# pfnet-research/superpixel-align

Measured on AMD Instinct MI355X. Metric: images/sec superpixel-align labelling (1024x2048), higher is better.
Workload: dtype f32 as 2 x f16 planes, f32 accumulate

## Files before the change

### include/spalign.h

```cpp
#ifndef SPALIGN_H
#define SPALIGN_H

#include <stddef.h>
#include <stdint.h>

#ifdef __cplusplus
extern "C" {
#endif

#define SPA_OK 0
#define SPA_ERR_ARG (-1)
#define SPA_ERR_HIP (-2)
#define SPA_ERR_NOGPU (-3)
#define SPA_ERR_LAYOUT (-4)
#define SPA_ERR_CAPACITY (-5)

#define SPA_ST_SLIC_EMPTY_SEGMENT 0x01u
#define SPA_ST_SLIC_UNCOVERED 0x02u
#define SPA_ST_CONN_OVERSIZE 0x04u
#define SPA_ST_POOL_SLOT_OVERFLOW 0x08u
#define SPA_ST_KMEANS_BARRIER 0x10u
#define SPA_ST_LABEL_RANGE 0x20u
#define SPA_ST_RNG_UNDERRUN 0x40u
#define SPA_ST_NP_SHUFFLE 0x80u
// ... 6 lines not shown
const char *spa_last_error(void);
int spa_ctx_create(int device, spa_ctx **out);
void spa_ctx_destroy(spa_ctx *ctx);
int spa_status(spa_ctx *ctx, uint32_t *status_host, void *stream);
int spa_status_peek_async(spa_ctx *ctx, uint32_t *status_pinned, void *stream);
int spa_status_take_async(spa_ctx *ctx, uint32_t *status_pinned, void *stream);

int spa_prof_enable(spa_ctx *ctx, int on);
int spa_prof_slots(void);
const char *spa_prof_name(int slot);
int spa_prof_read(spa_ctx *ctx, int slot, double *total_ms_host, int *launches_host);
int spa_debug_peek(spa_ctx *ctx, int which, size_t offset, size_t bytes, void *host);
int spa_ws_generation(spa_ctx *ctx);
int spa_debug_set(spa_ctx *ctx, int32_t key, int32_t value);
int spa_wino4_tile_decode(int32_t B, int32_t H, int32_t W, int32_t dilation, int32_t interleaved, int64_t t, int32_t *out);
int spa_debug_lds_probe(spa_ctx *ctx, float *out, int32_t n_wg, int32_t steps, int32_t mode, void *stream);

int spa_drn_normalise(spa_ctx *ctx, const float *x, int32_t B, int32_t H, int32_t W, void *out,
                      int32_t out_dtype, const double *mean3_host, const double *std3_host, void *stream);
int spa_bias_act(spa_ctx *ctx, void *y, int32_t dtype, int64_t rows, int32_t C, const void *bias,
                 const void *residual, int32_t relu, void *stream);
int spa_bias_act_amax(spa_ctx *ctx, float *y, int64_t rows, int32_t C, const float *bias,
                      const float *residual, int32_t relu, void *amax, void *stream);

int spa_drn_stem_d(spa_ctx *ctx, const float *x, int32_t B, int32_t H, int32_t W,
                   const float *w0, const float *b0, const float *w1, const float *b1,
                   const double *mean3_host, const double *std3_host, void *y, int32_t out_dtype,
                   float *xn_scratch, void *stream);

int spa_conv3x3_bf16(spa_ctx *ctx, const void *x, int32_t B, int32_t H, int32_t W, int32_t Cin,
// ... 281 lines not shown
```

### superpixel-align_amd/_lib.py

```python
import ctypes
import os
import subprocess

_HERE = os.path.dirname(os.path.abspath(__file__))
LIB_PATH = os.environ.get('SPA_LIB_PATH') or os.path.join(_HERE, 'libspalign.so')
_LIB = None

SPA_OK = 0
STATUS_BITS = {
    0x01: 'SLIC: a seed lost all of its pixels (NaN centre, dead for the rest of the sweeps, as in scikit-image)',
    0x02: 'SLIC: a pixel fell outside every 2S search window',
    0x04: 'connectivity: a component reached max_size (cut in BFS order by the exact replay path)',
    0x08: 'mean pooling: more than 16 superpixels touch one feature pixel',
    0x10: 'k-means: grid barrier timed out',
    0x20: 'a superpixel label outside [0, n_labels) was met',
    0x40: 'anchor selection: the device random stream ran dry',
    0x80: 'k-means initial assignment on the device: more than 65 536 points at or below the median weight',
}

INFO_BITS = 0x01 | 0x04

c_i32 = ctypes.c_int32
c_i64 = ctypes.c_int64
c_f32 = ctypes.c_float
# ... 44 lines not shown
    'spa_bias_act_amax': (ctypes.c_int, [c_p, c_p, c_i64, c_i32, c_p, c_p, c_i32, c_p, c_p]),
    'spa_drn_stem_d_amax': (ctypes.c_int, [c_p, c_p, c_i32, c_i32, c_i32, c_p, c_p, c_p, c_p, c_p, c_p, c_p, c_p, c_p, c_p]),
    'spa_drn_stem_c_amax': (ctypes.c_int, [c_p, c_p, c_i32, c_i32, c_i32, c_p, c_p, c_p, c_p, c_p, c_p, c_p, c_p, c_p, c_p, c_p]),
    'spa_drn_stem_c_bf16': (ctypes.c_int, [c_p, c_p, c_i32, c_i32, c_i32, c_p, c_p, c_p, c_p, c_p, c_p, c_p, c_p, c_p, c_p]),
    'spa_conv_small_f16s': (ctypes.c_int, [c_p, c_p, c_i32, c_i32, c_i32, c_i32, c_p, c_f32, c_i32, c_i32, c_i32, c_p, c_p, c_i32, c_p, c_p, c_p, c_p, c_p]),
    'spa_drn_layer2_f16s': (ctypes.c_int, [c_p, c_p, c_i32, c_i32, c_i32, c_p, c_f32, c_p, c_p, c_p, c_p, c_p]),
    'spa_drn_layer2_f32': (ctypes.c_int, [c_p, c_p, c_i32, c_i32, c_i32, c_p, c_p, c_p, c_p]),
    'spa_conv3x3_s2_f32': (ctypes.c_int, [c_p, c_p, c_i32, c_i32, c_i32, c_i32, c_p, c_i32, c_i32, c_p, c_i32, c_p, c_p, c_p]),
    'spa_amax_f32': (ctypes.c_int, [c_p, c_p, c_i64, c_p, c_p]),
    'spa_conv3x3_wino4_f16s': (ctypes.c_int, [c_p, c_p, c_i32, c_i32, c_i32, c_i32, c_p, c_p, c_i32, c_p, c_p, c_i32, c_i32, c_p, c_p, c_p, c_p, c_p, c_p]),
    'spa_resize_bicubic_u8': (ctypes.c_int, [c_p, c_p, c_i32, c_i32, c_i32, c_i32, c_i32, c_i32, c_p, c_p]),
    'spa_resize_cvcubic_u8': (ctypes.c_int, [c_p, c_p, c_i32, c_i32, c_i32, c_i32, c_i32, c_i32, c_p, c_p]),
    'spa_debug_peek': (ctypes.c_int, [c_p, ctypes.c_int, ctypes.c_size_t, ctypes.c_size_t, c_p]),
    'spa_debug_set': (ctypes.c_int, [c_p, ctypes.c_int32, ctypes.c_int32]),
    'spa_wino4_tile_decode': (ctypes.c_int, [c_i32, c_i32, c_i32, c_i32, c_i32, c_i64, ctypes.POINTER(ctypes.c_int32)]),
    'spa_ws_generation': (ctypes.c_int, [c_p]),
    'spa_debug_lds_probe': (ctypes.c_int, [c_p, c_p, c_i32, c_i32, c_i32, c_p]),
    'spa_slic_make_plan':(ctypes.c_int, [c_i32, c_i32, c_i32, ctypes.POINTER(SlicPlan)]),
    'spa_rgb2lab': (ctypes.c_int, [c_p, c_p, c_i32, c_i32, c_i32, c_f32, c_p, c_p]),
    'spa_slic_core': (ctypes.c_int, [c_p, c_p, c_i32, c_i32, c_i32, c_i32, c_i32, c_p, c_p, c_p]),
    'spa_enforce_connectivity': (ctypes.c_int, [c_p, c_p, c_i32, c_i32, c_i32, c_i32, c_i32, c_p,
                                                c_p, c_p]),
    'spa_slic': (ctypes.c_int, [c_p, c_p, c_i32, c_i32, c_i32, c_i32, c_f32, c_i32, c_p, c_p, c_p]),
    'spa_felzenszwalb': (ctypes.c_int, [c_p, c_p, c_i32, c_i32, c_i32, c_f64, c_f64, c_i32, c_p, c_p, c_p]),
    'spa_rgb2lab_u8_f64': (ctypes.c_int, [c_p, c_p, c_i32, c_i32, c_i32, c_f64, c_p, c_p]),
    'spa_slic_core_f64': (ctypes.c_int, [c_p, c_p, c_i32, c_i32, c_i32, c_i32, c_i32, c_p, c_p, c_p]),
    'spa_slic_u8': (ctypes.c_int, [c_p, c_p, c_i32, c_i32, c_i32, c_i32, c_f64, c_i32, c_p, c_p, c_p]),
    'spa_felzenszwalb_u8': (ctypes.c_int, [c_p, c_p, c_i32, c_i32, c_i32, c_f64, c_f64, c_i32, c_p, c_p, c_p]),
    'spa_overlap_refine': (ctypes.c_int, [c_p, c_p, c_p, c_i32, c_i64, c_i32, c_f64, c_p, c_p]),
    'spa_segment_offsets':(ctypes.c_int, [c_p, c_p, c_i32, c_p, c_p]),
# ... 111 lines not shown
```

### superpixel-align_amd/csrc/spa_common.h

```cpp
#pragma once
#include <hip/hip_runtime.h>
#include <stdint.h>
#include <stdio.h>
#include <string.h>

#include "../../include/spalign.h"

#define SPA_WAVE 64

void spa_set_error(const char *fmt, ...);

#define SPA_HIP(call)                                                                  \
    do {                                                                               \
        hipError_t e_ = (call);                                                        \
        if (e_ != hipSuccess) {                                                        \
            spa_set_error("%s failed: %s (%s:%d)", #call, hipGetErrorString(e_),      \
                          __FILE__, __LINE__);                                         \
            return SPA_ERR_HIP;                                                        \
        }                                                                              \
    } while (0)

#define SPA_ARG(cond)                                                                  \
    do {                                                                               \
        if (!(cond)) {                                                                 \
// ... 80 lines not shown
    hipStream_t aux[2];
    hipEvent_t ev_fork, ev_join[2];
    int aux_ready;
    int km_attr_done[2];
    int conn_attr_done;
    int conn_claim_ready;
    size_t conn_claim_bytes;
    int upd_wg_per_cu, upd_wg_per_cu8;
    int slic_force_general;
    int zero_line_ready, conv_attr_done, conv32_attr_done, fz_attr_done, gemm16_attr_done, gemm16s_attr_done, gemm16p_attr_done, nprng_attr_done;
    int rng_seeded;
    int ws_generation;
    int dbg_slic_ldsx;
    int convp_on;
    int wino_operands;
    int convs2_on;
    int convs2_attr_done;
    int rs_key[4], rs_ks[2];
};

#ifdef __HIPCC__
__device__ __forceinline__ unsigned spa_split16_pair(float x0, float x1, float sc, unsigned &l)
{
    unsigned h, lo;
    asm("v_fma_mixlo_f16 %0, %2, %4, 0 op_sel_hi:[0,0,0]\n\t"
        "v_fma_mixhi_f16 %0, %3, %4, 0 op_sel_hi:[0,0,0]\n\t"
        "v_fma_mixlo_f16 %1, %2, %4, -%0 op_sel_hi:[0,0,1]\n\t"
        "v_fma_mixhi_f16 %1, %3, %4, -%0 op_sel:[0,0,1] op_sel_hi:[0,0,1]"
        : "=&v"(h), "=&v"(lo) : "v"(x0), "v"(x1), "v"(sc));
    l = lo;
// ... 75 lines not shown
```

### superpixel-align_amd/csrc/spa_ctx.hip

```cpp
#include <math.h>
#include <stdarg.h>
#include <stdlib.h>

#include "spa_common.h"

static thread_local char g_err[512] = "";

void spa_set_error(const char *fmt, ...)
{
    va_list ap;
    va_start(ap, fmt);
    vsnprintf(g_err, sizeof(g_err), fmt, ap);
    va_end(ap);
}

extern "C" const char *spa_last_error(void) { return g_err; }
extern "C" int spa_version(void) { return 100; }

extern "C" int spa_ctx_create(int device, spa_ctx **out)
{
    SPA_ARG(out != nullptr);
    int n = 0;
    if (hipGetDeviceCount(&n) != hipSuccess || n <= 0) {
        spa_set_error("no HIP device visible: libspalign has no CPU fallback");
// ... 4 lines not shown
    SPA_HIP(hipSetDevice(device));
    hipDeviceProp_t prop;
    SPA_HIP(hipGetDeviceProperties(&prop, device));
    if (strncmp(prop.gcnArchName, "gfx950", 6) != 0) {
        spa_set_error("device %d is %s; libspalign is built for gfx950 (MI355X) only", device,
                      prop.gcnArchName);
        return SPA_ERR_NOGPU;
    }
    spa_ctx *ctx = (spa_ctx *)calloc(1, sizeof(spa_ctx));
    ctx->device = device;
    ctx->n_cu = prop.multiProcessorCount;
    if (const char *e = getenv("SPA_SLIC_GENERAL")) ctx->slic_force_general = atoi(e) != 0;
    ctx->convp_on = getenv("SPA_CONVP") ? atoi(getenv("SPA_CONVP")) != 0 : 1;
    ctx->convs2_on = 1;
    ctx->wino_operands = 2;
    SPA_HIP(hipMalloc((void **)&ctx->d_status, 32 * sizeof(uint32_t)));
    SPA_HIP(hipMemset(ctx->d_status, 0, 32 * sizeof(uint32_t)));
    *out = ctx;
    return SPA_OK;
}

extern "C" void spa_ctx_destroy(spa_ctx *ctx)
{
    if (!ctx) return;
    for (int i = 0; i < PROF_SLOTS; ++i) {
        for (int j = 0; j < ctx->prof_cap[i]; ++j) (void)hipEventDestroy(ctx->prof_ev[i][j]);
        free(ctx->prof_ev[i]);
    }
    for (int i = 0; i < WS_COUNT; ++i)
        if (ctx->ws[i]) (void)hipFree(ctx->ws[i]);
// ... 240 lines not shown
    *(float4 *)(out + ((long long)blockIdx.x * 256 + tid) * 4) = r;
}

extern "C" int spa_debug_lds_probe(spa_ctx *ctx, float *out, int32_t n_wg, int32_t steps, int32_t mode, void *stream)
{
    SPA_ARG(ctx && out && n_wg > 0 && steps > 0 && steps <= 32 && mode >= 0 && mode <= 2);
    hipLaunchKernelGGL(k_debug_lds_probe, dim3((unsigned)n_wg), dim3(256), 0, spa_stream(stream), out, steps, mode, 0.731f);
    SPA_LAUNCH_CHECK();
    return SPA_OK;
}

extern "C" int spa_ws_generation(spa_ctx *ctx) { return ctx ? ctx->ws_generation : -1; }

extern "C" int spa_debug_set(spa_ctx *ctx, int32_t key, int32_t value)
{
    SPA_ARG(ctx && (key == 1 || key == 2 || key == 3 || key == 4) && (value == 0 || value == 1 || (key == 4 && value == 2)));
    if (key == 1) ctx->convp_on = value;
    else if (key == 4) ctx->wino_operands = value;
    else if (key == 3) ctx->convs2_on = value;
    else {
#ifdef SPA_DIAG
        ctx->dbg_slic_ldsx = value;
#else
        SPA_ARG(!"spa_debug_set key 2 (the reproducer variant of k_slic_assign) exists in diagnostic builds only: make EXTRA=-DSPA_DIAG");
#endif
    }
    return SPA_OK;
}

extern "C" int spa_debug_peek(spa_ctx *ctx, int which, size_t offset, size_t bytes, void *host)
{
    if (which == -1) which = WS_DEBUG;
// ... 6 lines not shown
```

### superpixel-align_amd/csrc/spa_gemm16.hip

```cpp
#include "spa_common.h"
#include "spa_wino_dev.h"

typedef _Float16 f16x8 __attribute__((ext_vector_type(8)));
typedef float f32x4 __attribute__((ext_vector_type(4)));
typedef float f32x8 __attribute__((ext_vector_type(8)));

#define G16_THREADS 512
__device__ __forceinline__ void g16_lds_barrier()
{
    __builtin_amdgcn_sched_barrier(0);
    asm volatile("s_waitcnt lgkmcnt(0)\n\ts_barrier" ::: "memory");
    __builtin_amdgcn_sched_barrier(0);
}

template <int BM, int BN>
__global__ __launch_bounds__(G16_THREADS, 2) void k_gemm_f16x3(const char *__restrict__ X, const char *__restrict__ Wt,
                                                            float *__restrict__ Y, int rows_per_z, int Cin, int Cout,
                                                            int ntiles, int total_tiles, int zcount, long long xz,
                                                            long long wz, long long yz, const unsigned *__restrict__ amax)
{
    extern __shared__ __attribute__((aligned(1024))) char lds16[];
    const int tid = threadIdx.x, lane = tid & 63;
    const int wave = __builtin_amdgcn_readfirstlane(tid >> 6);
    const long long all_tiles = (long long)zcount * total_tiles;
// ... 130 lines not shown
        for (int j = 0; j < NJ; ++j) {
            const long long row = (long long)e_r0 + wn * (NJ * 16) + j * 16 + (lane & 15);
#pragma unroll
            for (int i = 0; i < MI; ++i) {
                const int c = e_n0 + wm * WROWS + i * 16 + (lane >> 4) * 4;
                *(float4 *)(e_y + row * Cout + c) = make_float4(acc[i][j][0], acc[i][j][1], acc[i][j][2], acc[i][j][3]);
            }
        }
        if (!more) break;
    }
}

template <int BM, int BN, bool PLANES = false>
__global__ __launch_bounds__(G16_THREADS) void k_gemm_f16x3_stag(const char *__restrict__ X, const char *__restrict__ Wt,
                                                                 float *__restrict__ Y, int rows_per_z, int Cin, int Cout,
                                                                 int ntiles, int total_tiles, int zcount, long long xz,
                                                                 long long wz, long long yz, const unsigned *__restrict__ amax)
{
    extern __shared__ __attribute__((aligned(1024))) char lds16[];
    const int tid = threadIdx.x, lane = tid & 63;
    const int wave = __builtin_amdgcn_readfirstlane(tid >> 6);
    const bool late = wave >= 4;
    const int all_i = zcount * total_tiles, gstep = (int)gridDim.x;
    const int nwg = total_tiles;
    float sb = 0.f;
    if (!PLANES) {
        const unsigned bits = *amax;
        int e = (int)(bits >> 23) - 127;
        e = e < -100 ? -100 : (e > 100 ? 100 : e);
        sb = __uint_as_float((unsigned)(127 + 14 - (bits == 0u ? 0 : e)) << 23);
    }
    int r0 = 0, n0 = 0, zz = 0;
// ... 15 lines not shown
    constexpr int WN = 4;
    constexpr int MI = BM == 256 ? 8 : 4;
    constexpr int NJ = BN / WN / 16;
    constexpr int WROWS = MI * 16;
    constexpr int RS = 3;
    static_assert(BM / WROWS * WN == 8, "8 waves");
    static_assert(MI * NJ <= 63, "vmcnt range");
    static_assert(RS <= NJ && MI == 8, "split schedule: 4 element pairs over 8 groups of matrix instructions");

    char *wbuf = lds16, *xbuf = lds16 + 2 * (BM * 128);
    const int sub = lane >> 3, cs = lane & 7;
    const int chunk_byte = (cs ^ sub) << 4;
    const int nk = Cin / 32;
    const char *s_w = nullptr, *s_x = nullptr;
    const unsigned lane_off = (unsigned)((wave * 8 + sub) * Cin * 4 + chunk_byte);
    auto stage_bases = [&]() {
        s_w = Wt + ((long long)zz * wz + (long long)n0 * Cin) * 4;
        s_x = X + ((long long)zz * xz + (long long)r0 * Cin) * 4;
    };
    auto stage = [&](int t, int buf) {
        const char *wk = s_w + (long long)t * 128;
        char *dw = wbuf + buf * (BM * 128) + wave * 1024;
#pragma unroll
        for (int r = 0; r < BM / 64; ++r)
            __builtin_amdgcn_global_load_lds((const __attribute__((address_space(1))) void *)(wk + (long long)r * 64 * Cin * 4 + lane_off),
                                             (__attribute__((address_space(3))) void *)(dw + r * 8192), 16, 0, 0);
        const char *xk = s_x + (long long)t * 128;
        char *dx = xbuf + buf * (BN * 128) + wave * 1024;
#pragma unroll
        for (int r = 0; r < BN / 64; ++r)
            __builtin_amdgcn_global_load_lds((const __attribute__((address_space(1))) void *)(xk + (long long)r * 64 * Cin * 4 + lane_off),
                                             (__attribute__((address_space(3))) void *)(dx + r * 8192), 16, 0, 0);
    };
    const int wm = wave / WN, wn = wave % WN;
    const int frow = lane & 15, fk = lane >> 4;
    if ((int)blockIdx.x >= all_i) return;
    const int my_tiles = (all_i - (int)blockIdx.x + gstep - 1) / gstep;
    const int S = my_tiles * nk;

    int s_vid = (int)blockIdx.x, s_t = 0, s_q = 0;
    locate(s_vid);
    stage_bases();
    int c_r0 = r0, c_n0 = n0, c_z = zz, c_t = 0, c_vid = s_vid;
    float c_zscale = zscale_s;
    auto stage_next = [&]() {
        if (s_q < S) {
// ... 41 lines not shown
        auto split_l = [&](int j, int e) {
            const float x0 = e < 2 ? ra[j][2 * e] : rb[j][2 * e - 4], x1 = e < 2 ? ra[j][2 * e + 1] : rb[j][2 * e - 3];
            lu[j][e] = wino_split_l(x0, x1, sc, hu[j][e]);
        };
        if (PLANES) {
#pragma unroll
            for (int j = 0; j < NJ; ++j) { hu[j] = __builtin_bit_cast(u32x4, ra[j]); lu[j] = __builtin_bit_cast(u32x4, rb[j]); }
        } else {
#pragma unroll
            for (int j = 0; j < RS; ++j)
#pragma unroll
                for (int e = 0; e < 4; ++e) { split_h(j, e); split_l(j, e); }
        }
        if (late) asm volatile("s_waitcnt vmcnt(0)" ::: "memory");
        g16_lds_barrier();
        float *const e_y = Y + (long long)c_z * yz + ((long long)c_r0 + wn * (NJ * 16) + (lane & 15)) * Cout + (c_n0 + wm * WROWS + (lane >> 4) * 4);
        auto store_acc = [&](int i, int j) {
            *(float4 *)(e_y + (long long)(j * 16) * Cout + i * 16) = make_float4(acc[i][j][0], acc[i][j][1], acc[i][j][2], acc[i][j][3]);
            acc[i][j] = (f32x4){0.f, 0.f, 0.f, 0.f};
        };
#pragma unroll
        for (int j = 0; j < NJ; ++j) {
            const f16x8 phj = __builtin_bit_cast(f16x8, hu[j]), plj = __builtin_bit_cast(f16x8, lu[j]);
#pragma unroll
            for (int i = 0; i < MI; ++i) {
                acc[i][j] = __builtin_amdgcn_mfma_f32_16x16x32_f16(wl[i], phj, acc[i][j], 0, 0, 0);
                acc[i][j] = __builtin_amdgcn_mfma_f32_16x16x32_f16(wh[i], plj, acc[i][j], 0, 0, 0);
                acc[i][j] = __builtin_amdgcn_mfma_f32_16x16x32_f16(wh[i], phj, acc[i][j], 0, 0, 0);
                if (!PLANES && j + RS < NJ) { if ((i & 1) == 0) split_h(j + RS, i >> 1); else split_l(j + RS, i >> 1); }
                __builtin_amdgcn_sched_barrier(0);
            }
        }
        if (++c_t == nk) {
// ... 12 lines not shown
        }
        if (!late) {
            if (stored) asm volatile("s_waitcnt vmcnt(%0)" ::"n"(MI * NJ) : "memory");
            else asm volatile("s_waitcnt vmcnt(0)" ::: "memory");
            g16_lds_barrier();
        } else if (q + 1 < S) {
            g16_lds_barrier();
        }
        stored = false;
    }
}

int gemm_f16x3_tile(int32_t Cout) { return Cout % 256 == 0 ? 256 : 128; }

int gemm_f16x3_raw(spa_ctx *ctx, const float *x, long long rows, int32_t Cin, const void *wt, int32_t Cout, float *y,
                   void *stream, int zcount, const void *amax, int planes)
{
    SPA_ARG(ctx && x && wt && y && amax && rows > 0 && rows % 256 == 0 && rows < (1ll << 31) && zcount == 36);
    SPA_ARG(Cin % 32 == 0 && Cout % 128 == 0);
    SPA_ARG(((uintptr_t)x % 16) == 0 && ((uintptr_t)wt % 16) == 0 && ((uintptr_t)y % 16) == 0);
    hipStream_t s = spa_stream(stream);
    const int bm = gemm_f16x3_tile(Cout), bn = bm;
    SPA_ARG(!planes || bm == 256);
    const int ntiles = Cout / bm;
    const long long total = rows / bn * ntiles;
    SPA_ARG(total < (1ll << 31));
    const size_t lds = 2 * (size_t)(bm + bn) * 128;
    SpaProfScope prof_(ctx, bm == 256 ? PROF_DRN_GEMM16 : PROF_DRN_GEMM16_N, s);
    const int per_cu = lds > 80 * 1024 ? 1 : 2;
    long long grid = (long long)ctx->n_cu * per_cu;
    if (grid > total * zcount) grid = total * zcount;
    if (bm == 256) {
        if (!ctx->gemm16s_attr_done) {
            SPA_HIP(hipFuncSetAttribute((const void *)k_gemm_f16x3_stag<256, 256>, hipFuncAttributeMaxDynamicSharedMemorySize, 2 * 512 * 128));
            ctx->gemm16s_attr_done = 1;
        }
        if (planes) {
            if (!ctx->gemm16p_attr_done) {
                SPA_HIP(hipFuncSetAttribute((const void *)k_gemm_f16x3_stag<256, 256, true>, hipFuncAttributeMaxDynamicSharedMemorySize, 2 * 512 * 128));
                ctx->gemm16p_attr_done = 1;
            }
            hipLaunchKernelGGL((k_gemm_f16x3_stag<256, 256, true>), dim3((unsigned)grid), dim3(G16_THREADS), lds, s, (const char *)x, (const char *)wt, y,
                               (int)rows, Cin, Cout, ntiles, (int)total, zcount, rows * Cin, (long long)Cout * Cin, rows * Cout, (const unsigned *)amax);
        } else
        hipLaunchKernelGGL((k_gemm_f16x3_stag<256, 256>), dim3((unsigned)grid), dim3(G16_THREADS), lds, s, (const char *)x, (const char *)wt, y,
                           (int)rows, Cin, Cout, ntiles, (int)total, zcount, rows * Cin, (long long)Cout * Cin, rows * Cout, (const unsigned *)amax);
    } else {
        if (!ctx->gemm16_attr_done) {
            SPA_HIP(hipFuncSetAttribute((const void *)k_gemm_f16x3<128, 128>, hipFuncAttributeMaxDynamicSharedMemorySize, 2 * 256 * 128));
            ctx->gemm16_attr_done = 1;
        }
        hipLaunchKernelGGL((k_gemm_f16x3<128, 128>), dim3((unsigned)grid), dim3(G16_THREADS), lds, s, (const char *)x, (const char *)wt, y,
                           (int)rows, Cin, Cout, ntiles, (int)total, zcount, rows * Cin, (long long)Cout * Cin, rows * Cout, (const unsigned *)amax);
    }
    SPA_LAUNCH_CHECK();
    return SPA_OK;
}
```

### superpixel-align_amd/csrc/spa_wino.hip

```cpp
#include "spa_common.h"
#include "spa_wino_dev.h"

int conv1x1_f32_raw(spa_ctx *ctx, const float *x, long long rows, int32_t Cin, const float *wt, int32_t Cout,
                    float *y, void *stream, int zcount);

extern "C" int spa_wino4_tile_decode(int32_t B, int32_t H, int32_t W, int32_t dilation, int32_t interleaved, int64_t t, int32_t *out)
{
    SPA_ARG(out && B > 0 && H > 0 && W > 0 && dilation >= 1);
    WinoGeom g;
    wino4_geom(B, H, W, dilation, &g);
    SPA_ARG(t >= 0 && t < g.T);
    g.interleaved = interleaved != 0;
    wino_tile(g, t, out[0], out[1], out[2], out[3], out[4]);
    return SPA_OK;
}


__device__ __forceinline__ float4 f4add(float4 a, float4 b) { return make_float4(a.x + b.x, a.y + b.y, a.z + b.z, a.w + b.w); }
__device__ __forceinline__ float4 f4sub(float4 a, float4 b) { return make_float4(a.x - b.x, a.y - b.y, a.z - b.z, a.w - b.w); }

__device__ __forceinline__ long long wino_block()
{
    const long long nb = gridDim.x, id = blockIdx.x;
    const long long q = nb / 8, rem = nb % 8, xcd = id % 8, idx = id / 8;
    return (xcd < rem ? xcd * (q + 1) : rem * (q + 1) + (xcd - rem) * q) + idx;
}


__global__ __launch_bounds__(256) void k_wino_in(const float *__restrict__ X, float *__restrict__ V, WinoGeom g, int C,
                                                 long long Tpad)
{
// ... 123 lines not shown
        if (residual)
            hipLaunchKernelGGL(k_wino_out<1>, dim3((unsigned)((n + 255) / 256)), dim3(256), 0, s, (const float *)m_scratch, y,
                               bias, residual, g, Cout, Tpad, relu);
        else
            hipLaunchKernelGGL(k_wino_out<0>, dim3((unsigned)((n + 255) / 256)), dim3(256), 0, s, (const float *)m_scratch, y,
                               bias, residual, g, Cout, Tpad, relu);
    }
    SPA_LAUNCH_CHECK();
    return SPA_OK;
}



template <typename V, bool PLANES = false>
__global__ __launch_bounds__(256) void k_wino4_in(const float *__restrict__ X, float *__restrict__ Vout, WinoGeom g, int C,
                                                  long long Tpad, const unsigned *__restrict__ amax = nullptr)
{
    constexpr int VN = sizeof(V) / 4;
    const int c2 = C / VN;
    const long long id = wino_block() * 256 + threadIdx.x;
    if (id >= g.T * c2) return;
    const long long t = id / c2;
    const int c = (int)(id - t * c2) * VN;
    int b, sy, sx, ty, tx;
    wino_tile(g, t, b, sy, sx, ty, tx);
    V r[6][6];
#pragma unroll
    for (int a = 0; a < 6; ++a) {
        const int y = sy + (4 * ty - 1 + a) * g.d;
        V dv[6];
#pragma unroll
        for (int j = 0; j < 6; ++j) {
            const int x = sx + (4 * tx - 1 + j) * g.d;
            const bool ok = y >= 0 && y < g.H && x >= 0 && x < g.W;
            dv[j] = ok ? *(const V *)(X + (((long long)b * g.H + y) * g.W + x) * C + c) : wino_zero<V>();
        }
        wino4_bt(dv, r[a]);
    }
#pragma unroll
    for (int j = 0; j < 6; ++j) {
        const V col[6] = {r[0][j], r[1][j], r[2][j], r[3][j], r[4][j], r[5][j]};
        V o[6];
        wino4_bt(col, o);
#pragma unroll
        for (int i = 0; i < 6; ++i) {
            if constexpr (PLANES) {
                static_assert(sizeof(V) == 16, "a thread owns half an 8-channel chunk");
                const float sc = wino_pow2(14 - wino_amax_exp(*amax) - wino4_psum(i * 6 + j));
                const unsigned h0 = wino_split_h(o[i].x, o[i].y, sc), h1 = wino_split_h(o[i].z, o[i].w, sc);
                const unsigned l0 = wino_split_l(o[i].x, o[i].y, sc, h0), l1 = wino_split_l(o[i].z, o[i].w, sc, h1);
                const bool odd = (c >> 2) & 1;
                const unsigned r0 = wino_lane_swap(odd ? h0 : l0), r1 = wino_lane_swap(odd ? h1 : l1);
                float *chunk = Vout + ((long long)(i * 6 + j) * Tpad + t) * C + (c & ~7);
                *((uint4 *)chunk + (odd ? 1 : 0)) = odd ? make_uint4(r0, r1, l0, l1) : make_uint4(h0, h1, r0, r1);
            } else {
                *(V *)(Vout + ((long long)(i * 6 + j) * Tpad + t) * C + c) = o[i];
            }
        }
    }
}

template <int HAS_RES, typename V>
__global__ __launch_bounds__(256) void k_wino4_out(const float *__restrict__ M, float *__restrict__ Y,
                                                   const float *__restrict__ bias, const float *__restrict__ R,
                                                   WinoGeom g, int K, long long Tpad, int relu)
{
    constexpr int VN = sizeof(V) / 4;
    const int k2 = K / VN;
    const long long id = wino_block() * 256 + threadIdx.x;
    if (id >= g.T * k2) return;
    const long long t = id / k2;
// ... 41 lines not shown
        m = max(max(m, __float_as_uint(v.x) & 0x7fffffffu), max(__float_as_uint(v.y) & 0x7fffffffu,
                max(__float_as_uint(v.z) & 0x7fffffffu, __float_as_uint(v.w) & 0x7fffffffu)));
    }
    for (int o = 32; o > 0; o >>= 1) m = max(m, (unsigned)__shfl_xor((int)m, o));
    if ((threadIdx.x & 63) == 0) red[threadIdx.x >> 6] = m;
    __syncthreads();
    if (threadIdx.x == 0) {
        m = max(max(red[0], red[1]), max(red[2], red[3]));
        if (m > *(volatile unsigned *)amax) atomicMax(amax, m);
    }
}

template <int HAS_RES, typename V = float4>
__global__ __launch_bounds__(256, 2) void k_wino4_out_s(const float *__restrict__ M, float *__restrict__ Y,
                                                     const float *__restrict__ bias, const float *__restrict__ R,
                                                     WinoGeom g, int K, long long Tpad, int relu, WinoScale cs,
                                                     const unsigned *__restrict__ amax_in, unsigned *__restrict__ amax_out)
{
    constexpr int VN = sizeof(V) / 4;
    const int k2 = K / VN;
    const long long id = wino_block() * 256 + threadIdx.x;
    unsigned mx = 0;
    if (id < g.T * k2) {
        const long long t = id / k2;
        const int k = (int)(id - t * k2) * VN;
        int b, sy, sx, ty, tx;
        wino_tile(g, t, b, sy, sx, ty, tx);
        const float inv = wino_pow2(wino_amax_exp(*amax_in) - 14);
        V s[4][6];
#pragma unroll
        for (int j = 0; j < 6; ++j) {
            V col[6];
#pragma unroll
            for (int i = 0; i < 6; ++i)
                col[i] = (cs.c[i * 6 + j] * inv) * wino_nt_load((const V *)(M + ((long long)(i * 6 + j) * Tpad + t) * K + k));
            V o[4];
            wino4_at(col, o);
#pragma unroll
            for (int i = 0; i < 4; ++i) s[i][j] = o[i];
        }
        const V bv = *(const V *)(bias + k);
#pragma unroll
        for (int i = 0; i < 4; ++i) {
            const int y = sy + (4 * ty + i) * g.d;
            V o[4];
            wino4_at(s[i], o);
            if (y >= g.H) continue;
#pragma unroll
            for (int j = 0; j < 4; ++j) {
                const int x = sx + (4 * tx + j) * g.d;
// ... 22 lines not shown

extern "C" int spa_conv3x3_wino4_f32(spa_ctx *ctx, const float *x, int32_t B, int32_t H, int32_t W, int32_t Cin,
                                     const float *u, int32_t Cout, const float *bias, const float *residual,
                                     int32_t relu, int32_t dilation, float *v_scratch, float *m_scratch, float *y,
                                     void *stream)
{
    SPA_ARG(ctx && x && u && bias && y && v_scratch && m_scratch && B > 0 && H > 0 && W > 0 && dilation >= 1);
    SPA_ARG(Cin % 32 == 0 && Cout % 64 == 0);
    SPA_ARG((((uintptr_t)x | (uintptr_t)u | (uintptr_t)y | (uintptr_t)bias | (uintptr_t)residual | (uintptr_t)v_scratch |
              (uintptr_t)m_scratch) % 16) == 0);
    hipStream_t s = spa_stream(stream);
    WinoGeom g;
    wino4_geom(B, H, W, dilation, &g);
    g.interleaved = ctx->wino_operands >= 1 && wino_interleave(dilation);
    const long long Tpad = (g.T + 255) / 256 * 256;
    SPA_ARG(g.T * (Cin > Cout ? Cin : Cout) / 2 < (1ll << 31) * 256);
    {
        SpaProfScope prof_(ctx, PROF_WINO_IN, s);
        const long long n = g.T * (Cin / 4);
        hipLaunchKernelGGL((k_wino4_in<float4, false>), dim3((unsigned)((n + 255) / 256)), dim3(256), 0, s, x, v_scratch, g, Cin, Tpad,
                           (const unsigned *)nullptr);
    }
    {
        int rc = conv1x1_f32_raw(ctx, v_scratch, Tpad, Cin, u, Cout, m_scratch, stream, 36);
        if (rc != SPA_OK) return rc;
    }
    {
        SpaProfScope prof_(ctx, PROF_WINO_OUT, s);
        const long long n = g.T * (Cout / 4);
        if (residual)
            hipLaunchKernelGGL((k_wino4_out<1, float4>), dim3((unsigned)((n + 255) / 256)), dim3(256), 0, s, (const float *)m_scratch, y,
                               bias, residual, g, Cout, Tpad, relu);
        else
            hipLaunchKernelGGL((k_wino4_out<0, float4>), dim3((unsigned)((n + 255) / 256)), dim3(256), 0, s, (const float *)m_scratch, y,
                               bias, residual, g, Cout, Tpad, relu);
    }
    SPA_LAUNCH_CHECK();
    return SPA_OK;
}

int gemm_f16x3_raw(spa_ctx *ctx, const float *x, long long rows, int32_t Cin, const void *wt, int32_t Cout, float *y,
                   void *stream, int zcount, const void *amax, int planes);
int gemm_f16x3_tile(int32_t Cout);

extern "C" int spa_amax_f32(spa_ctx *ctx, const float *x, int64_t n, void *amax, void *stream)
{
    SPA_ARG(ctx && x && amax && n > 0 && n % 4 == 0 && ((uintptr_t)x % 16) == 0);
    hipStream_t s = spa_stream(stream);
    spa_zero_word(amax, s);
    long long blocks = (n / 4 + 255) / 256;
    if (blocks > 4096) blocks = 4096;
    hipLaunchKernelGGL(k_amax, dim3((unsigned)blocks), dim3(256), 0, s, (const float4 *)x, (long long)(n / 4), (unsigned *)amax);
    SPA_LAUNCH_CHECK();
    return SPA_OK;
}

extern "C" int spa_conv3x3_wino4_f16s(spa_ctx *ctx, const float *x, int32_t B, int32_t H, int32_t W, int32_t Cin,
                                      const void *u2, const float *cs, int32_t Cout, const float *bias,
                                      const float *residual, int32_t relu, int32_t dilation, const void *amax_in,
                                      void *amax_out, void *v_scratch, float *m_scratch, float *y, void *stream)
{
    SPA_ARG(ctx && x && u2 && cs && bias && y && v_scratch && m_scratch && amax_in && B > 0 && H > 0 && W > 0 && dilation >= 1);
    SPA_ARG(Cin % 32 == 0 && Cout % 128 == 0);
    SPA_ARG((((uintptr_t)x | (uintptr_t)u2 | (uintptr_t)y | (uintptr_t)bias | (uintptr_t)residual | (uintptr_t)v_scratch |
              (uintptr_t)m_scratch) % 16) == 0);
    hipStream_t s = spa_stream(stream);
    WinoGeom g;
    wino4_geom(B, H, W, dilation, &g);
    g.interleaved = ctx->wino_operands >= 1 && wino_interleave(dilation);
    const int planes = ctx->wino_operands >= 2 && gemm_f16x3_tile(Cout) == 256 && Cout >= 512;
    const long long Tpad = (g.T + 255) / 256 * 256;
    SPA_ARG(g.T * (Cin > Cout ? Cin : Cout) / 4 < (1ll << 31) * 256);
    WinoScale sc;
    for (int i = 0; i < 36; ++i) sc.c[i] = cs[i];
    if (amax_out) spa_zero_word(amax_out, s);
    {
        SpaProfScope prof_(ctx, PROF_WINO_IN, s);
        const long long n = g.T * (Cin / 4);
        if (planes)
            hipLaunchKernelGGL((k_wino4_in<float4, true>), dim3((unsigned)((n + 255) / 256)), dim3(256), 0, s, x, (float *)v_scratch, g, Cin, Tpad,
                               (const unsigned *)amax_in);
        else
            hipLaunchKernelGGL((k_wino4_in<float4, false>), dim3((unsigned)((n + 255) / 256)), dim3(256), 0, s, x, (float *)v_scratch, g, Cin, Tpad,
                               (const unsigned *)nullptr);
    }
    {
        int rc = gemm_f16x3_raw(ctx, (const float *)v_scratch, Tpad, Cin, u2, Cout, m_scratch, stream, 36, amax_in, planes);
        if (rc != SPA_OK) return rc;
    }
    {
        SpaProfScope prof_(ctx, PROF_WINO_OUT, s);
        const long long n = g.T * (Cout / 4);
        if (residual)
            hipLaunchKernelGGL((k_wino4_out_s<1>), dim3((unsigned)((n + 255) / 256)), dim3(256), 0, s, (const float *)m_scratch, y,
                               bias, residual, g, Cout, Tpad, relu, sc, (const unsigned *)amax_in, (unsigned *)amax_out);
        else
            hipLaunchKernelGGL((k_wino4_out_s<0>), dim3((unsigned)((n + 255) / 256)), dim3(256), 0, s, (const float *)m_scratch, y,
                               bias, residual, g, Cout, Tpad, relu, sc, (const unsigned *)amax_in, (unsigned *)amax_out);
    }
    SPA_LAUNCH_CHECK();
    return SPA_OK;
}
```

### superpixel-align_amd/csrc/spa_wino_dev.h

```cpp
#pragma once
#include "spa_common.h"

struct WinoGeom { int B, H, W, d, th, tw; long long T; int interleaved; };
typedef float wino_v4 __attribute__((ext_vector_type(4)));
__device__ __forceinline__ float4 wino_nt_load(const float4 *p) { const wino_v4 v = __builtin_nontemporal_load((const wino_v4 *)p); return make_float4(v[0], v[1], v[2], v[3]); }

__host__ __device__ __forceinline__ void wino_tile(const WinoGeom &g, long long t, int &b, int &sy, int &sx, int &ty, int &tx)
{
    if (g.interleaved) {
        const int rw = g.tw * g.d;
        const int gx = (int)(t % rw); t /= rw;
        sx = gx % g.d; tx = gx / g.d;
        ty = (int)(t % g.th); t /= g.th;
        sy = (int)(t % g.d);
        b = (int)(t / g.d);
        return;
    }
    tx = (int)(t % g.tw); t /= g.tw;
    ty = (int)(t % g.th); t /= g.th;
    sx = (int)(t % g.d); t /= g.d;
    sy = (int)(t % g.d);
    b = (int)(t / g.d);
}

__device__ __forceinline__ unsigned wino_absmax_bits(float4 v) { return max(max(__float_as_uint(v.x) & 0x7fffffffu, __float_as_uint(v.y) & 0x7fffffffu), max(__float_as_uint(v.z) & 0x7fffffffu, __float_as_uint(v.w) & 0x7fffffffu)); }
__device__ __forceinline__ float4 operator+(float4 a, float4 b) { return make_float4(a.x + b.x, a.y + b.y, a.z + b.z, a.w + b.w); }
__device__ __forceinline__ float4 operator-(float4 a, float4 b) { return make_float4(a.x - b.x, a.y - b.y, a.z - b.z, a.w - b.w); }
__device__ __forceinline__ float4 operator*(float s, float4 a) { return make_float4(s * a.x, s * a.y, s * a.z, s * a.w); }
template <typename V> __device__ __forceinline__ V wino_zero();
template <> __device__ __forceinline__ float4 wino_zero<float4>() { return make_float4(0.f, 0.f, 0.f, 0.f); }
__device__ __forceinline__ float4 wino_relu(float4 v) { return make_float4(fmaxf(v.x, 0.f), fmaxf(v.y, 0.f), fmaxf(v.z, 0.f), fmaxf(v.w, 0.f)); }

template <typename V>
__device__ __forceinline__ void wino4_bt(const V (&x)[6], V (&y)[6])
{
    y[0] = 2.0f * (x[0] + x[4]) + 3.0f * (x[3] - x[1]) - 4.0f * x[2];
    y[1] = 2.0f * (x[4] - x[1]) + x[2] + 5.0f * x[3];
    y[2] = 5.0f * x[2] - 2.0f * (x[1] + x[4]) - x[3];
// ... 60 lines not shown
```

Before: 448.6.

## Store Winograd V/M operands block-major in 256-tile blocks for the f16x3 GEMM

Introduces a WinoLayout abstraction (planes, block-major, tile-major) for the Winograd transformed input and GEMM output buffers. When the GEMM tile is 256, the input transform, GEMM loads and stores, and output transform now use a block-major layout that keeps all 36 z-planes of a 256-tile block contiguous. This is meant to improve locality between the transform kernels and the GEMM, so that the 36 scattered plane strides per tile become one compact block. Layout offsets are computed with an extra divide/mod per row, and a diagnostic knob and a host offset helper are added for testing.

After: 451.9, median of 4. No clear change (+0.7%).

```diff
diff --git a/include/spalign.h b/include/spalign.h
--- a/include/spalign.h
+++ b/include/spalign.h
@@ -44,6 +44,7 @@
 int spa_ws_generation(spa_ctx *ctx);
 int spa_debug_set(spa_ctx *ctx, int32_t key, int32_t value);
 int spa_wino4_tile_decode(int32_t B, int32_t H, int32_t W, int32_t dilation, int32_t interleaved, int64_t t, int32_t *out);
+int64_t spa_wino4_layout_offset(int32_t layout, int64_t Tpad, int32_t C, int32_t z, int64_t t, int32_t c);
 int spa_debug_lds_probe(spa_ctx *ctx, float *out, int32_t n_wg, int32_t steps, int32_t mode, void *stream);
 
 int spa_drn_normalise(spa_ctx *ctx, const float *x, int32_t B, int32_t H, int32_t W, void *out,
diff --git a/superpixel-align_amd/_lib.py b/superpixel-align_amd/_lib.py
--- a/superpixel-align_amd/_lib.py
+++ b/superpixel-align_amd/_lib.py
@@ -82,6 +82,7 @@
     'spa_debug_peek': (ctypes.c_int, [c_p, ctypes.c_int, ctypes.c_size_t, ctypes.c_size_t, c_p]),
     'spa_debug_set': (ctypes.c_int, [c_p, ctypes.c_int32, ctypes.c_int32]),
     'spa_wino4_tile_decode': (ctypes.c_int, [c_i32, c_i32, c_i32, c_i32, c_i32, c_i64, ctypes.POINTER(ctypes.c_int32)]),
+    'spa_wino4_layout_offset': (ctypes.c_int64, [c_i32, c_i64, c_i32, c_i32, c_i64, c_i32]),
     'spa_ws_generation': (ctypes.c_int, [c_p]),
     'spa_debug_lds_probe': (ctypes.c_int, [c_p, c_p, c_i32, c_i32, c_i32, c_p]),
     'spa_slic_make_plan':(ctypes.c_int, [c_i32, c_i32, c_i32, ctypes.POINTER(SlicPlan)]),
diff --git a/superpixel-align_amd/csrc/spa_common.h b/superpixel-align_amd/csrc/spa_common.h
--- a/superpixel-align_amd/csrc/spa_common.h
+++ b/superpixel-align_amd/csrc/spa_common.h
@@ -118,6 +118,7 @@
     int dbg_slic_ldsx;
     int convp_on;
     int wino_operands;
+    int dbg_wino_layout;
     int convs2_on;
     int convs2_attr_done;
     int rs_key[4], rs_ks[2];
diff --git a/superpixel-align_amd/csrc/spa_ctx.hip b/superpixel-align_amd/csrc/spa_ctx.hip
--- a/superpixel-align_amd/csrc/spa_ctx.hip
+++ b/superpixel-align_amd/csrc/spa_ctx.hip
@@ -42,6 +42,7 @@
     ctx->convp_on = getenv("SPA_CONVP") ? atoi(getenv("SPA_CONVP")) != 0 : 1;
     ctx->convs2_on = 1;
     ctx->wino_operands = 2;
+    ctx->dbg_wino_layout = -1;
     SPA_HIP(hipMalloc((void **)&ctx->d_status, 32 * sizeof(uint32_t)));
     SPA_HIP(hipMemset(ctx->d_status, 0, 32 * sizeof(uint32_t)));
     *out = ctx;
@@ -312,8 +313,15 @@
 
 extern "C" int spa_debug_set(spa_ctx *ctx, int32_t key, int32_t value)
 {
-    SPA_ARG(ctx && (key == 1 || key == 2 || key == 3 || key == 4) && (value == 0 || value == 1 || (key == 4 && value == 2)));
+    SPA_ARG(ctx && (key == 1 || key == 2 || key == 3 || key == 4 || key == 5) && (value == 0 || value == 1 || (key == 4 && value == 2) || (key == 5 && value >= -1 && value < 9)));
     if (key == 1) ctx->convp_on = value;
+    else if (key == 5) {
+#ifdef SPA_DIAG
+        ctx->dbg_wino_layout = value;
+#else
+        SPA_ARG(!"spa_debug_set key 5 (the row layouts of the Winograd operands) exists in diagnostic builds only: make EXTRA=-DSPA_DIAG");
+#endif
+    }
     else if (key == 4) ctx->wino_operands = value;
     else if (key == 3) ctx->convs2_on = value;
     else {
diff --git a/superpixel-align_amd/csrc/spa_gemm16.hip b/superpixel-align_amd/csrc/spa_gemm16.hip
--- a/superpixel-align_amd/csrc/spa_gemm16.hip
+++ b/superpixel-align_amd/csrc/spa_gemm16.hip
@@ -168,8 +168,8 @@
 template <int BM, int BN, bool PLANES = false>
 __global__ __launch_bounds__(G16_THREADS) void k_gemm_f16x3_stag(const char *__restrict__ X, const char *__restrict__ Wt,
                                                                  float *__restrict__ Y, int rows_per_z, int Cin, int Cout,
-                                                                 int ntiles, int total_tiles, int zcount, long long xz,
-                                                                 long long wz, long long yz, const unsigned *__restrict__ amax)
+                                                                 int ntiles, int total_tiles, int zcount, WinoLayout lx,
+                                                                 long long wz, WinoLayout ly, const unsigned *__restrict__ amax)
 {
     extern __shared__ __attribute__((aligned(1024))) char lds16[];
     const int tid = threadIdx.x, lane = tid & 63;
@@ -215,9 +215,18 @@
     const int nk = Cin / 32;
     const char *s_w = nullptr, *s_x = nullptr;
     const unsigned lane_off = (unsigned)((wave * 8 + sub) * Cin * 4 + chunk_byte);
+#ifdef SPA_DIAG
+    const int xp = (int)wino_pitch(lx, Cin) * 4;
+    const long long yp = wino_pitch(ly, Cout);
+    const unsigned lane_off_x = (unsigned)((wave * 8 + sub) * xp + chunk_byte);
+#else
+    const int xp = Cin * 4;
+    const long long yp = Cout;
+    const unsigned lane_off_x = lane_off;
+#endif
     auto stage_bases = [&]() {
         s_w = Wt + ((long long)zz * wz + (long long)n0 * Cin) * 4;
-        s_x = X + ((long long)zz * xz + (long long)r0 * Cin) * 4;
+        s_x = X + wino_off(lx, zz, r0, Cin) * 4;
     };
     auto stage = [&](int t, int buf) {
         const char *wk = s_w + (long long)t * 128;
@@ -230,7 +239,7 @@
         char *dx = xbuf + buf * (BN * 128) + wave * 1024;
 #pragma unroll
         for (int r = 0; r < BN / 64; ++r)
-            __builtin_amdgcn_global_load_lds((const __attribute__((address_space(1))) void *)(xk + (long long)r * 64 * Cin * 4 + lane_off),
+            __builtin_amdgcn_global_load_lds((const __attribute__((address_space(1))) void *)(xk + (long long)r * 64 * xp + lane_off_x),
                                              (__attribute__((address_space(3))) void *)(dx + r * 8192), 16, 0, 0);
     };
     const int wm = wave / WN, wn = wave % WN;
@@ -302,9 +311,9 @@
         }
         if (late) asm volatile("s_waitcnt vmcnt(0)" ::: "memory");
         g16_lds_barrier();
-        float *const e_y = Y + (long long)c_z * yz + ((long long)c_r0 + wn * (NJ * 16) + (lane & 15)) * Cout + (c_n0 + wm * WROWS + (lane >> 4) * 4);
+        float *const e_y = Y + wino_off(ly, c_z, c_r0, Cout) + (long long)(wn * (NJ * 16) + (lane & 15)) * yp + (c_n0 + wm * WROWS + (lane >> 4) * 4);
         auto store_acc = [&](int i, int j) {
-            *(float4 *)(e_y + (long long)(j * 16) * Cout + i * 16) = make_float4(acc[i][j][0], acc[i][j][1], acc[i][j][2], acc[i][j][3]);
+            *(float4 *)(e_y + (long long)(j * 16) * yp + i * 16) = make_float4(acc[i][j][0], acc[i][j][1], acc[i][j][2], acc[i][j][3]);
             acc[i][j] = (f32x4){0.f, 0.f, 0.f, 0.f};
         };
 #pragma unroll
@@ -347,7 +356,7 @@
 int gemm_f16x3_tile(int32_t Cout) { return Cout % 256 == 0 ? 256 : 128; }
 
 int gemm_f16x3_raw(spa_ctx *ctx, const float *x, long long rows, int32_t Cin, const void *wt, int32_t Cout, float *y,
-                   void *stream, int zcount, const void *amax, int planes)
+                   void *stream, int zcount, const void *amax, int planes, WinoLayout lx, WinoLayout ly)
 {
     SPA_ARG(ctx && x && wt && y && amax && rows > 0 && rows % 256 == 0 && rows < (1ll << 31) && zcount == 36);
     SPA_ARG(Cin % 32 == 0 && Cout % 128 == 0);
@@ -355,6 +364,9 @@
     hipStream_t s = spa_stream(stream);
     const int bm = gemm_f16x3_tile(Cout), bn = bm;
     SPA_ARG(!planes || bm == 256);
+#ifndef SPA_DIAG
+    SPA_ARG(lx.rows_per_block % 256 == 0 && ly.rows_per_block % 256 == 0);
+#endif
     const int ntiles = Cout / bm;
     const long long total = rows / bn * ntiles;
     SPA_ARG(total < (1ll << 31));
@@ -374,11 +386,12 @@
                 ctx->gemm16p_attr_done = 1;
             }
             hipLaunchKernelGGL((k_gemm_f16x3_stag<256, 256, true>), dim3((unsigned)grid), dim3(G16_THREADS), lds, s, (const char *)x, (const char *)wt, y,
-                               (int)rows, Cin, Cout, ntiles, (int)total, zcount, rows * Cin, (long long)Cout * Cin, rows * Cout, (const unsigned *)amax);
+                               (int)rows, Cin, Cout, ntiles, (int)total, zcount, lx, (long long)Cout * Cin, ly, (const unsigned *)amax);
         } else
         hipLaunchKernelGGL((k_gemm_f16x3_stag<256, 256>), dim3((unsigned)grid), dim3(G16_THREADS), lds, s, (const char *)x, (const char *)wt, y,
-                           (int)rows, Cin, Cout, ntiles, (int)total, zcount, rows * Cin, (long long)Cout * Cin, rows * Cout, (const unsigned *)amax);
+                           (int)rows, Cin, Cout, ntiles, (int)total, zcount, lx, (long long)Cout * Cin, ly, (const unsigned *)amax);
     } else {
+        SPA_ARG(lx.rows_per_block == rows && ly.rows_per_block == rows);
         if (!ctx->gemm16_attr_done) {
             SPA_HIP(hipFuncSetAttribute((const void *)k_gemm_f16x3<128, 128>, hipFuncAttributeMaxDynamicSharedMemorySize, 2 * 256 * 128));
             ctx->gemm16_attr_done = 1;
diff --git a/superpixel-align_amd/csrc/spa_wino.hip b/superpixel-align_amd/csrc/spa_wino.hip
--- a/superpixel-align_amd/csrc/spa_wino.hip
+++ b/superpixel-align_amd/csrc/spa_wino.hip
@@ -15,6 +15,12 @@
     return SPA_OK;
 }
 
+extern "C" int64_t spa_wino4_layout_offset(int32_t layout, int64_t Tpad, int32_t C, int32_t z, int64_t t, int32_t c)
+{
+    if (layout < 0 || layout >= WINO_LAYOUTS || Tpad <= 0 || Tpad % 256 || Tpad >= (1ll << 31) || C <= 0 || z < 0 || z >= 36 || t < 0 ||
+        t >= Tpad || c < 0 || c >= C) return -1;
+    return wino_off(wino_layout(layout, Tpad, C), z, t, C) + c;
+}
 
 __device__ __forceinline__ float4 f4add(float4 a, float4 b) { return make_float4(a.x + b.x, a.y + b.y, a.z + b.z, a.w + b.w); }
 __device__ __forceinline__ float4 f4sub(float4 a, float4 b) { return make_float4(a.x - b.x, a.y - b.y, a.z - b.z, a.w - b.w); }
@@ -168,7 +174,7 @@
 
 template <typename V, bool PLANES = false>
 __global__ __launch_bounds__(256) void k_wino4_in(const float *__restrict__ X, float *__restrict__ Vout, WinoGeom g, int C,
-                                                  long long Tpad, const unsigned *__restrict__ amax = nullptr)
+                                                  WinoLayout L, const unsigned *__restrict__ amax = nullptr)
 {
     constexpr int VN = sizeof(V) / 4;
     const int c2 = C / VN;
@@ -178,6 +184,7 @@
     const int c = (int)(id - t * c2) * VN;
     int b, sy, sx, ty, tx;
     wino_tile(g, t, b, sy, sx, ty, tx);
+    float *const vrow = Vout + wino_row(L, t, C);
     V r[6][6];
 #pragma unroll
     for (int a = 0; a < 6; ++a) {
@@ -205,10 +212,10 @@
                 const unsigned l0 = wino_split_l(o[i].x, o[i].y, sc, h0), l1 = wino_split_l(o[i].z, o[i].w, sc, h1);
                 const bool odd = (c >> 2) & 1;
                 const unsigned r0 = wino_lane_swap(odd ? h0 : l0), r1 = wino_lane_swap(odd ? h1 : l1);
-                float *chunk = Vout + ((long long)(i * 6 + j) * Tpad + t) * C + (c & ~7);
+                float *chunk = vrow + (i * 6 + j) * L.z_stride + (c & ~7);
                 *((uint4 *)chunk + (odd ? 1 : 0)) = odd ? make_uint4(r0, r1, l0, l1) : make_uint4(h0, h1, r0, r1);
             } else {
-                *(V *)(Vout + ((long long)(i * 6 + j) * Tpad + t) * C + c) = o[i];
+                *(V *)(vrow + (i * 6 + j) * L.z_stride + c) = o[i];
             }
         }
     }
@@ -280,7 +287,7 @@
 template <int HAS_RES, typename V = float4>
 __global__ __launch_bounds__(256, 2) void k_wino4_out_s(const float *__restrict__ M, float *__restrict__ Y,
                                                      const float *__restrict__ bias, const float *__restrict__ R,
-                                                     WinoGeom g, int K, long long Tpad, int relu, WinoScale cs,
+                                                     WinoGeom g, int K, WinoLayout L, int relu, WinoScale cs,
                                                      const unsigned *__restrict__ amax_in, unsigned *__restrict__ amax_out)
 {
     constexpr int VN = sizeof(V) / 4;
@@ -293,13 +300,14 @@
         int b, sy, sx, ty, tx;
         wino_tile(g, t, b, sy, sx, ty, tx);
         const float inv = wino_pow2(wino_amax_exp(*amax_in) - 14);
+        const float *const mrow = M + wino_row(L, t, K) + k;
         V s[4][6];
 #pragma unroll
         for (int j = 0; j < 6; ++j) {
             V col[6];
 #pragma unroll
             for (int i = 0; i < 6; ++i)
-                col[i] = (cs.c[i * 6 + j] * inv) * wino_nt_load((const V *)(M + ((long long)(i * 6 + j) * Tpad + t) * K + k));
+                col[i] = (cs.c[i * 6 + j] * inv) * wino_nt_load((const V *)(mrow + (i * 6 + j) * L.z_stride));
             V o[4];
             wino4_at(col, o);
 #pragma unroll
@@ -352,12 +360,12 @@
     wino4_geom(B, H, W, dilation, &g);
     g.interleaved = ctx->wino_operands >= 1 && wino_interleave(dilation);
     const long long Tpad = (g.T + 255) / 256 * 256;
-    SPA_ARG(g.T * (Cin > Cout ? Cin : Cout) / 2 < (1ll << 31) * 256);
+    SPA_ARG(g.T * (Cin > Cout ? Cin : Cout) / 2 < (1ll << 31) * 256 && Tpad < (1ll << 31));
     {
         SpaProfScope prof_(ctx, PROF_WINO_IN, s);
         const long long n = g.T * (Cin / 4);
-        hipLaunchKernelGGL((k_wino4_in<float4, false>), dim3((unsigned)((n + 255) / 256)), dim3(256), 0, s, x, v_scratch, g, Cin, Tpad,
-                           (const unsigned *)nullptr);
+        hipLaunchKernelGGL((k_wino4_in<float4, false>), dim3((unsigned)((n + 255) / 256)), dim3(256), 0, s, x, v_scratch, g, Cin,
+                           wino_layout(WINO_PLANES, Tpad, Cin), (const unsigned *)nullptr);
     }
     {
         int rc = conv1x1_f32_raw(ctx, v_scratch, Tpad, Cin, u, Cout, m_scratch, stream, 36);
@@ -378,7 +386,7 @@
 }
 
 int gemm_f16x3_raw(spa_ctx *ctx, const float *x, long long rows, int32_t Cin, const void *wt, int32_t Cout, float *y,
-                   void *stream, int zcount, const void *amax, int planes);
+                   void *stream, int zcount, const void *amax, int planes, WinoLayout lx, WinoLayout ly);
 int gemm_f16x3_tile(int32_t Cout);
 
 extern "C" int spa_amax_f32(spa_ctx *ctx, const float *x, int64_t n, void *amax, void *stream)
@@ -408,7 +416,12 @@
     g.interleaved = ctx->wino_operands >= 1 && wino_interleave(dilation);
     const int planes = ctx->wino_operands >= 2 && gemm_f16x3_tile(Cout) == 256 && Cout >= 512;
     const long long Tpad = (g.T + 255) / 256 * 256;
-    SPA_ARG(g.T * (Cin > Cout ? Cin : Cout) / 4 < (1ll << 31) * 256);
+    SPA_ARG(g.T * (Cin > Cout ? Cin : Cout) / 4 < (1ll << 31) * 256 && Tpad < (1ll << 31));
+    int kind_v = gemm_f16x3_tile(Cout) == 256 ? WINO_BLOCK_MAJOR : WINO_PLANES, kind_m = kind_v;
+#ifdef SPA_DIAG
+    if (gemm_f16x3_tile(Cout) == 256 && ctx->dbg_wino_layout >= 0) { kind_v = ctx->dbg_wino_layout % 3; kind_m = ctx->dbg_wino_layout / 3; }
+#endif
+    const WinoLayout lv = wino_layout(kind_v, Tpad, Cin), lm = wino_layout(kind_m, Tpad, Cout);
     WinoScale sc;
     for (int i = 0; i < 36; ++i) sc.c[i] = cs[i];
     if (amax_out) spa_zero_word(amax_out, s);
@@ -416,14 +429,14 @@
         SpaProfScope prof_(ctx, PROF_WINO_IN, s);
         const long long n = g.T * (Cin / 4);
         if (planes)
-            hipLaunchKernelGGL((k_wino4_in<float4, true>), dim3((unsigned)((n + 255) / 256)), dim3(256), 0, s, x, (float *)v_scratch, g, Cin, Tpad,
+            hipLaunchKernelGGL((k_wino4_in<float4, true>), dim3((unsigned)((n + 255) / 256)), dim3(256), 0, s, x, (float *)v_scratch, g, Cin, lv,
                                (const unsigned *)amax_in);
         else
-            hipLaunchKernelGGL((k_wino4_in<float4, false>), dim3((unsigned)((n + 255) / 256)), dim3(256), 0, s, x, (float *)v_scratch, g, Cin, Tpad,
+            hipLaunchKernelGGL((k_wino4_in<float4, false>), dim3((unsigned)((n + 255) / 256)), dim3(256), 0, s, x, (float *)v_scratch, g, Cin, lv,
                                (const unsigned *)nullptr);
     }
     {
-        int rc = gemm_f16x3_raw(ctx, (const float *)v_scratch, Tpad, Cin, u2, Cout, m_scratch, stream, 36, amax_in, planes);
+        int rc = gemm_f16x3_raw(ctx, (const float *)v_scratch, Tpad, Cin, u2, Cout, m_scratch, stream, 36, amax_in, planes, lv, lm);
         if (rc != SPA_OK) return rc;
     }
     {
@@ -431,10 +444,10 @@
         const long long n = g.T * (Cout / 4);
         if (residual)
             hipLaunchKernelGGL((k_wino4_out_s<1>), dim3((unsigned)((n + 255) / 256)), dim3(256), 0, s, (const float *)m_scratch, y,
-                               bias, residual, g, Cout, Tpad, relu, sc, (const unsigned *)amax_in, (unsigned *)amax_out);
+                               bias, residual, g, Cout, lm, relu, sc, (const unsigned *)amax_in, (unsigned *)amax_out);
         else
             hipLaunchKernelGGL((k_wino4_out_s<0>), dim3((unsigned)((n + 255) / 256)), dim3(256), 0, s, (const float *)m_scratch, y,
-                               bias, residual, g, Cout, Tpad, relu, sc, (const unsigned *)amax_in, (unsigned *)amax_out);
+                               bias, residual, g, Cout, lm, relu, sc, (const unsigned *)amax_in, (unsigned *)amax_out);
     }
     SPA_LAUNCH_CHECK();
     return SPA_OK;
diff --git a/superpixel-align_amd/csrc/spa_wino_dev.h b/superpixel-align_amd/csrc/spa_wino_dev.h
--- a/superpixel-align_amd/csrc/spa_wino_dev.h
+++ b/superpixel-align_amd/csrc/spa_wino_dev.h
@@ -22,6 +22,24 @@
     sy = (int)(t % g.d);
     b = (int)(t / g.d);
 }
+
+enum { WINO_PLANES = 0, WINO_BLOCK_MAJOR = 1, WINO_TILE_MAJOR = 2, WINO_LAYOUTS = 3 };
+struct WinoLayout { long long block_stride, z_stride; int rows_per_block; };
+__host__ __device__ __forceinline__ WinoLayout wino_layout(int kind, long long Tpad, int C)
+{
+    WinoLayout L;
+    if (kind == WINO_TILE_MAJOR) { L.block_stride = 36ll * C; L.z_stride = C; L.rows_per_block = 1; }
+    else if (kind == WINO_BLOCK_MAJOR) { L.block_stride = 36ll * 256 * C; L.z_stride = 256ll * C; L.rows_per_block = 256; }
+    else { L.block_stride = 0; L.z_stride = Tpad * C; L.rows_per_block = (int)Tpad; }
+    return L;
+}
+__host__ __device__ __forceinline__ long long wino_row(const WinoLayout &L, long long t, int C)
+{
+    const unsigned blk = (unsigned)t / (unsigned)L.rows_per_block, r = (unsigned)t - blk * (unsigned)L.rows_per_block;
+    return (long long)blk * L.block_stride + (long long)r * C;
+}
+__host__ __device__ __forceinline__ long long wino_off(const WinoLayout &L, int z, long long t, int C) { return wino_row(L, t, C) + z * L.z_stride; }
+__host__ __device__ __forceinline__ long long wino_pitch(const WinoLayout &L, int C) { return L.rows_per_block == 1 ? L.block_stride : C; }
 
 __device__ __forceinline__ unsigned wino_absmax_bits(float4 v) { return max(max(__float_as_uint(v.x) & 0x7fffffffu, __float_as_uint(v.y) & 0x7fffffffu), max(__float_as_uint(v.z) & 0x7fffffffu, __float_as_uint(v.w) & 0x7fffffffu)); }
 __device__ __forceinline__ float4 operator+(float4 a, float4 b) { return make_float4(a.x + b.x, a.y + b.y, a.z + b.z, a.w + b.w); }
```
